# shangfuu/avse_challenge

Hardware: AMD Instinct MI355X
Metric: utterances/sec (3s@16kHz + 75 lip frames) (higher is better)
Workload: dtype fp32; 1 GPU; avse1 AV baseline train step (BASELINE configs[1]): HIP STFT front-end + AVNet (ResNet18 lip enc + TCN, dilated Conv2d audio net, LSTM fusion) fwd/bwd + Adam; global_batch=32, per_gpu_batch=32, seq_len=48000, stft_frames=376, lip_frames=75, lip_hw=96, parallelism=dp1, hip_graph=fwd+bwd+opt

## Files before the change

avse_challenge_amd/_lib.py:

```python
import ctypes
import os

import torch

_HERE = os.path.dirname(os.path.abspath(__file__))
LIB_PATH = os.environ.get("AVSE_HIP_LIB", os.path.join(_HERE, "libavse_hip.so"))

c_i64, c_i32, c_f32, c_vp = ctypes.c_int64, ctypes.c_int32, ctypes.c_float, ctypes.c_void_p

AVSE_F32, AVSE_BF16 = 0, 1


class ScanFwdArgs(ctypes.Structure):
    _fields_ = [
        ("batch", c_i64), ("dim", c_i64), ("seqlen", c_i64), ("dstate", c_i64),
        ("in_dtype", c_i32), ("delta_softplus", c_i32), ("reverse", c_i32),
        ("u", c_vp), ("u_bs", c_i64), ("u_ds", c_i64),
        ("delta", c_vp), ("delta_bs", c_i64), ("delta_ds", c_i64),
        ("A", c_vp),
        ("B", c_vp), ("B_bs", c_i64), ("B_ns", c_i64),
        ("C", c_vp), ("C_bs", c_i64), ("C_ns", c_i64),
        ("D", c_vp),
        ("z", c_vp), ("z_bs", c_i64), ("z_ds", c_i64),
        ("delta_bias", c_vp),
# ... 114 lines not shown
    "avse_prelu_gln_workspace_bytes": (c_i64, [c_i64, c_i64]),
    "avse_prelu_gln_fwd": (c_i32, [c_i64, c_i64, c_i64, c_vp, c_vp, c_vp, c_vp, c_f32, c_vp, c_vp, c_vp, c_vp]),
    "avse_prelu_gln_bwd": (c_i32, [c_i64, c_i64, c_i64] + [c_vp] * 11),
    "avse_prelu_gln_bwd_q": (c_i32, [c_i64, c_i64, c_i64] + [c_vp] * 7 + [c_i64] + [c_vp] * 6),
    "avse_dwconv_bwd_workspace_bytes": (c_i64, [c_i64, c_i64]),
    "avse_dwconv_fwd": (c_i32, [c_i64, c_i64, c_i64, c_i64, c_i64, c_vp, c_vp, c_vp, c_vp]),
    "avse_dwconv_bwd": (c_i32, [c_i64, c_i64, c_i64, c_i64, c_i64] + [c_vp] * 7),
    "avse_dwconv_gln_workspace_bytes": (c_i64, [c_i64, c_i64]),
    "avse_dwconv_gln_fwd": (c_i32, [c_i64] * 5 + [c_vp] * 5 + [c_f32] + [c_vp] * 5),
    "avse_dwconv_gln_fwd_q": (c_i32, [c_i64] * 5 + [c_vp] * 5 + [c_f32] + [c_vp] * 3 + [c_i64] + [c_vp] * 4),
    "avse_dwconv_gln_bwd": (c_i32, [c_i64] * 5 + [c_vp] * 14),
    "avse_lstm_padded_hidden": (c_i64, [c_i64]),
    "avse_lstm_group_size": (c_i64, [c_i64, c_i64]),
    "avse_lstm_group_workspace_bytes": (c_i64, [c_i64, c_i64]),
    "avse_lstm_group_capacity": (c_i64, [c_i64, c_i32]),
    "avse_lstm_fwd_group": (c_i32, [c_i64, c_i64, c_i64, c_i32, c_vp, c_vp, c_vp, c_i64, c_i64, c_vp, c_vp, c_vp, c_vp,
                                    c_vp]),
    "avse_lstm_bwd_group": (c_i32, [c_i64, c_i64, c_i64, c_i32, c_vp, c_i64, c_i64, c_vp, c_vp, c_vp, c_vp, c_vp, c_vp,
                                    c_vp]),
    "avse_lstm_fwd": (c_i32, [c_i64, c_i64, c_i64, c_i32, c_vp, c_vp, c_vp, c_i64, c_i64, c_vp, c_vp, c_vp]),
    "avse_lstm_bwd": (c_i32, [c_i64, c_i64, c_i64, c_i32, c_vp, c_i64, c_i64, c_vp, c_vp, c_vp, c_vp, c_vp]),
    "avse_gemm_bf16": (c_i32, [ctypes.POINTER(GemmBf16Args), c_vp]),
    "avse_gemm_f32s": (c_i32, [ctypes.POINTER(GemmF32sArgs), c_vp]),
    "avse_split16_planes": (c_i32, [c_i64, c_i64, c_i64, c_vp, c_i64, c_i64, c_vp, c_vp, c_vp, c_vp]),
    "avse_add_max": (c_i32, [c_i64, c_i64, c_i64, c_vp, c_vp, c_vp, c_vp, c_vp]),
    "avse_split16_planes_known": (c_i32, [c_i64, c_i64, c_i64, c_vp, c_i64, c_i64, c_vp, c_vp, c_vp, c_vp]),
    "avse_split16_planes_to": (c_i32, [c_i64, c_i64, c_i64, c_vp, c_i64, c_i64, c_vp, c_vp, c_i64, c_i64, c_vp, c_i32,
                                       c_vp]),
    "avse_dconv_wprep_bytes": (c_i64, []),
    "avse_split16": (c_i32, [c_i64, c_vp, c_vp, c_vp, c_vp]),
    "avse_split16_known": (c_i32, [c_i64, c_vp, c_vp, c_vp, c_vp]),
    "avse_dconv_wprep": (c_i32, [c_vp, c_i32, c_vp, c_vp, c_vp]),
    "avse_dconv_fwd": (c_i32, [c_i64, c_i64, c_i64, c_i64, c_vp, c_vp, c_vp, c_vp, c_vp, c_vp]),
    "avse_dconv_wgrad16_workspace_bytes": (c_i64, [c_i64, c_i64, c_i64]),
    "avse_dconv_wgrad16": (c_i32, [c_i64, c_i64, c_i64, c_i64, c_vp, c_vp, c_vp, c_vp, c_vp, c_vp, c_vp, c_vp]),
    "avse_conv1_fwd": (c_i32, [c_i64] * 3 + [c_vp] * 5),
    "avse_conv1_dgrad": (c_i32, [c_i64] * 3 + [c_vp] * 4),
    "avse_conv1_wgrad_workspace_bytes": (c_i64, [c_i64] * 3),
    "avse_conv1_wgrad": (c_i32, [c_i64] * 3 + [c_vp] * 6),
    "avse_convf_fwd": (c_i32, [c_i64] + [c_vp] * 5),
    "avse_convf_dgrad": (c_i32, [c_i64] + [c_vp] * 4),
    "avse_convf_wgrad_workspace_bytes": (c_i64, [c_i64]),
    "avse_convf_wgrad": (c_i32, [c_i64] + [c_vp] * 6),
    "avse_sconv_wprep_bytes": (c_i64, [c_i64, c_i64]),
    "avse_sconv_wprep": (c_i32, [c_i64, c_i64, c_vp, c_i32, c_vp, c_vp, c_vp]),
    "avse_sconv_fwd": (c_i32, [c_i64] * 6 + [c_vp] * 6),
    "avse_sconv_wgrad_workspace_bytes": (c_i64, [c_i64] * 6),
    "avse_sconv_wgrad": (c_i32, [c_i64] * 6 + [c_vp] * 7),
    "avse_sconv_dgrad2_supported": (c_i32, [c_i64] * 5),
    "avse_sconv_dgrad2": (c_i32, [c_i64] * 5 + [c_vp] * 6),
}

_lib = None


class HipLibraryError(RuntimeError):
    pass


ABI_VERSION = 2


def lib():
    global _lib
    if _lib is None:
        if not os.path.exists(LIB_PATH):
# ... 30 lines not shown
```

avse_challenge_amd/csrc/dconv.hip:

```cpp
#include <algorithm>

#include "common.h"

namespace avse {
namespace dcf {

typedef _Float16 half8 __attribute__((ext_vector_type(8)));
typedef float floatx16 __attribute__((ext_vector_type(16)));
typedef int i4_t __attribute__((ext_vector_type(4)));
typedef __attribute__((address_space(3))) void lds_void_t;

constexpr int C = 64, KS = 5, NQ = 4, TP = 256, THREADS = 256, WAVES = THREADS / 64;
constexpr int ROWB = 64;
constexpr int WIMG = KS * C * ROWB;
constexpr int NSTG = KS * NQ;
constexpr int MAXD = 16;
constexpr int XIMG_MAX = (TP + 8 * MAXD) * ROWB;
constexpr int STAGE = XIMG_MAX + WIMG;
constexpr int NBUF = 3;
constexpr int MAXP = (XIMG_MAX + WIMG) / 1024 / WAVES + 1;
static_assert(NBUF * STAGE <= 160 * 1024, "LDS");

__device__ inline int swz(int r) { return (r >> 2) & 3; }

// ... 457 lines not shown
        d[0] = uint4{hi[0], hi[1], hi[2], hi[3]};
        d[1] = uint4{hi[4], hi[5], hi[6], hi[7]};
        d[2] = uint4{lo[0], lo[1], lo[2], lo[3]};
        d[3] = uint4{lo[4], lo[5], lo[6], lo[7]};
    }
}

__global__ __launch_bounds__(1024) void wprep_kernel(const float* w, int transposed, uint32_t* maxbits, uint16_t* wq) {
    __shared__ uint32_t red[16];
    constexpr int TOT = C * C * KS * KS;
    float m = 0.f;
    for (int i = threadIdx.x; i < TOT; i += blockDim.x) m = fmaxf(m, fabsf(w[i]));
    uint32_t b = __float_as_uint(m);
    for (int o = 32; o >= 1; o >>= 1) b = max(b, (uint32_t)__shfl_xor((int)b, o, 64));
    if ((threadIdx.x & 63) == 0) red[threadIdx.x >> 6] = b;
    __syncthreads();
    b = 0;
    for (int k = 0; k < (int)(blockDim.x >> 6); ++k) b = max(b, red[k]);
    if (threadIdx.x == 0) maxbits[1] = b;
    const float sc = __builtin_ldexpf(1.f, split_exp(b));
    for (int e = threadIdx.x; e < TOT; e += blockDim.x) {
        const int c = e % 16, o = (e / 16) % C, kw = (e / (16 * C)) % KS, s = e / (16 * C * KS);
        const int kh = s / NQ, q = s % NQ, i = q * 16 + c;
        const float v = transposed ? w[((i * C + o) * KS + (KS - 1 - kh)) * KS + (KS - 1 - kw)]
                                   : w[((o * C + i) * KS + kh) * KS + kw];
        const float sv = v * sc;
        const _Float16 h = (_Float16)sv, l = (_Float16)(sv - (float)h);
        const int64_t row = ((int64_t)s * KS + kw) * C + o;
        wq[row * 32 + c] = __builtin_bit_cast(uint16_t, h);
        wq[row * 32 + 16 + c] = __builtin_bit_cast(uint16_t, l);
    }
}

}
}

using namespace avse::dcf;

extern "C" {

int64_t avse_dconv_wprep_bytes(void) { return (int64_t)NSTG * WIMG; }

int avse_split16(int64_t n_pix, const float* x, void* xq, uint32_t* maxbits, avse_stream_t stream) {
    if (!x || !xq || !maxbits) return AVSE_EINVAL;
    if (n_pix <= 0) return AVSE_ESHAPE;
    if (((uintptr_t)x & 15) || ((uintptr_t)xq & 15)) return AVSE_EALIGN;
    hipStream_t st = (hipStream_t)stream;
    if (hipMemsetAsync(maxbits, 0, 4, st) != hipSuccess) return AVSE_ELAUNCH;
    const int64_t n4 = n_pix * C / 4;
    hipLaunchKernelGGL(absmax_kernel, dim3((unsigned)std::max<int64_t>(1, std::min<int64_t>(AMAX_GRID, (n4 + AMAX_NT - 1) / AMAX_NT))),
                       dim3(AMAX_NT), 0, st, reinterpret_cast<const float4*>(x), n4, maxbits);
    AVSE_CHECK_LAUNCH();
    const int64_t nq = n_pix * NQ;
    const int blocks = (int)std::min<int64_t>((nq + 255) / 256, 8192);
    hipLaunchKernelGGL(split_kernel, dim3(blocks), dim3(256), 0, st, x, nq, maxbits, reinterpret_cast<uint4*>(xq));
    AVSE_CHECK_LAUNCH();
    return AVSE_OK;
}

int avse_split16_known(int64_t n_pix, const float* x, void* xq, const uint32_t* maxbits, avse_stream_t stream) {
    if (!x || !xq || !maxbits) return AVSE_EINVAL;
    if (n_pix <= 0) return AVSE_ESHAPE;
    if (((uintptr_t)x & 15) || ((uintptr_t)xq & 15)) return AVSE_EALIGN;
    const int64_t nq = n_pix * NQ;
    const int blocks = (int)std::min<int64_t>((nq + 255) / 256, 8192);
    hipLaunchKernelGGL(split_kernel, dim3(blocks), dim3(256), 0, (hipStream_t)stream, x, nq, maxbits,
                       reinterpret_cast<uint4*>(xq));
    AVSE_CHECK_LAUNCH();
    return AVSE_OK;
}

int avse_dconv_wprep(const float* w, int32_t transposed, void* wq, uint32_t* maxbits, avse_stream_t stream) {
    if (!w || !wq || !maxbits) return AVSE_EINVAL;
    hipLaunchKernelGGL(wprep_kernel, dim3(1), dim3(1024), 0, (hipStream_t)stream, w, transposed, maxbits,
                       reinterpret_cast<uint16_t*>(wq));
    AVSE_CHECK_LAUNCH();
    return AVSE_OK;
}

int64_t avse_dconv_wgrad16_workspace_bytes(int64_t N, int64_t H, int64_t W) {
    const int64_t chunks = N * ((H * W + WG_CHUNK - 1) / WG_CHUNK);
    return 4 * 2 * (int64_t)wgrad_ranges((int)std::min<int64_t>(chunks, 1 << 30)) * (KS * KS * C * C + C);
}

int avse_dconv_wgrad16(int64_t N, int64_t H, int64_t W, int64_t dil, const void* xq, const uint32_t* xmax,
                       const void* dyq, const uint32_t* dymax, float* dw, float* db, float* workspace,
                       avse_stream_t stream) {
    if (!xq || !xmax || !dyq || !dymax || !dw || !workspace) return AVSE_EINVAL;
    if (N <= 0 || H <= 0 || W < WG_CHUNK || (dil != 2 && dil != 4 && dil != 8 && dil != 16)) return AVSE_ESHAPE;
    if (N * H * W * 256 >= (1LL << 31) - 1024) return AVSE_ESHAPE;
    WArgs a;
    a.xq = xq;
    a.dyq = dyq;
    a.xmax = xmax;
    a.dymax = dymax;
    a.N = (int)N;
    a.H = (int)H;
    a.W = (int)W;
    a.cpi = (int)((H * W + WG_CHUNK - 1) / WG_CHUNK);
    a.chunks = (int)(N * a.cpi);
    a.ranges = wgrad_ranges(a.chunks);
    a.part = workspace;
    a.dbpart = db ? workspace + (int64_t)2 * a.ranges * KS * KS * C * C : nullptr;
    const dim3 grid((unsigned)(a.ranges * KS)), block(WTHREADS);
    hipStream_t st = (hipStream_t)stream;
    switch (dil) {
        case 2: hipLaunchKernelGGL(wgrad_kernel<2>, grid, block, 0, st, a); break;
        case 4: hipLaunchKernelGGL(wgrad_kernel<4>, grid, block, 0, st, a); break;
// ... 41 lines not shown
```

avse_challenge_amd/csrc/projgemm.hip:

```cpp
#include <algorithm>

#include "common.h"

namespace avse {
namespace pg {

typedef __bf16 bf16x8 __attribute__((ext_vector_type(8)));
typedef short s4_t __attribute__((ext_vector_type(4)));
typedef short s8_t __attribute__((ext_vector_type(8)));
typedef float floatx16 __attribute__((ext_vector_type(16)));
typedef __attribute__((address_space(3))) void lds_void_t;
typedef __attribute__((address_space(3))) s4_t lds_s4_t;

constexpr int BT = 256, THREADS = 512, WAVES = THREADS / 64;
constexpr int BK = 32;
constexpr int IMG = BT * BK * 2;
constexpr int STAGE = 2 * IMG;
constexpr int NBUF = 4, AHEAD = NBUF - 1;
constexpr int LWAVES = 4;
constexpr int PIECES = IMG / 1024 / LWAVES;
constexpr int LOADS = 2 * PIECES;
constexpr int RB = 2 * BK, CPR = BK / 8, RPL = 256 / RB;
static_assert(NBUF * STAGE <= 160 * 1024, "LDS");
static_assert(AHEAD >= 2 && AHEAD <= 4, "ring depth: stage s + 1 is issued before iteration s");
// ... 396 lines not shown
                            } else if (p + 7 < a.mp) {
                                reinterpret_cast<uint2*>(dst)[0] = uint2{v.x, v.y};
                                reinterpret_cast<uint2*>(dst)[1] = uint2{v.z, v.w};
                            } else {
                                const uint32_t u[4] = {v.x, v.y, v.z, v.w};
#pragma unroll
                                for (int e = 0; e < 8; ++e)
                                    if (p + e < a.mp) dst[e] = (uint16_t)(u[e >> 1] >> (16 * (e & 1)));
                            }
                        }
                    }
                    asm volatile("s_waitcnt lgkmcnt(0)" ::: "memory");
                }
            }
        }
#pragma unroll
        for (int i = 0; i < 4; ++i)
#pragma unroll
            for (int j = 0; j < 2; ++j)
#pragma unroll
                for (int e = 0; e < 16; ++e) acc[i][j][e] = 0.f;
    }
}

}
}

using namespace avse::pg;

struct PlanesArgs {
    const float* x;
    int64_t rows, r, c, bs, rs, hbs, hrs;
    int rpb;
    uint32_t* maxbits;
    _Float16* hi;
    _Float16* lo;
};

__device__ inline int64_t planes_row_off(const PlanesArgs& a, int64_t row) { return (row / a.r) * a.bs + (row % a.r) * a.rs; }
__device__ inline int64_t planes_out_off(const PlanesArgs& a, int64_t row) {
    return (row / a.r) * a.hbs + (row % a.r) * a.hrs;
}

constexpr int AM_NT = 1024, AM_GRID = 256;
template <bool VEC>
__global__ __launch_bounds__(AM_NT) void planes_absmax_kernel(PlanesArgs a, int64_t nrb) {
    __shared__ uint32_t red[AM_NT / 64];
    float m = 0.f;
    const int64_t c4 = VEC ? a.c / 4 : 0;
    for (int64_t rb = blockIdx.x; rb < nrb; rb += gridDim.x)
    for (int rr = 0; rr < a.rpb; ++rr) {
        const int64_t row = rb * a.rpb + rr;
        if (row >= a.rows) break;
        const float* xr = a.x + planes_row_off(a, row);
        if constexpr (VEC) {
            for (int64_t j0 = threadIdx.x; j0 < c4; j0 += 4 * AM_NT) {
                float4 v[4];
#pragma unroll
                for (int u = 0; u < 4; ++u)
                    v[u] = j0 + u * AM_NT < c4 ? reinterpret_cast<const float4*>(xr)[j0 + u * AM_NT] : make_float4(0.f, 0.f, 0.f, 0.f);
#pragma unroll
                for (int u = 0; u < 4; ++u)
                    m = fmaxf(m, fmaxf(fmaxf(fabsf(v[u].x), fabsf(v[u].y)), fmaxf(fabsf(v[u].z), fabsf(v[u].w))));
            }
        }
        for (int64_t i0 = 4 * c4 + threadIdx.x; i0 < a.c; i0 += 4 * AM_NT) {
            float v[4];
#pragma unroll
            for (int u = 0; u < 4; ++u) v[u] = i0 + u * AM_NT < a.c ? xr[i0 + u * AM_NT] : 0.f;
#pragma unroll
            for (int u = 0; u < 4; ++u) m = fmaxf(m, fabsf(v[u]));
        }
    }
    uint32_t v = __float_as_uint(m);
    for (int o = 32; o >= 1; o >>= 1) v = max(v, (uint32_t)__shfl_xor((int)v, o, 64));
    if ((threadIdx.x & 63) == 0) red[threadIdx.x >> 6] = v;
    __syncthreads();
    if (threadIdx.x == 0) {
        for (int k = 1; k < AM_NT / 64; ++k) v = max(v, red[k]);
        v = max(v, red[0]);
        if (v) atomicMax(a.maxbits, v);
    }
}

__device__ inline uint32_t split_pair(float x0, float x1, float sc, uint32_t& lo) {
    const float s0 = x0 * sc, s1 = x1 * sc;
    const _Float16 h0 = (_Float16)s0, h1 = (_Float16)s1;
    const _Float16 l0 = (_Float16)(s0 - (float)h0), l1 = (_Float16)(s1 - (float)h1);
    lo = (uint32_t)__builtin_bit_cast(uint16_t, l0) | ((uint32_t)__builtin_bit_cast(uint16_t, l1) << 16);
    return (uint32_t)__builtin_bit_cast(uint16_t, h0) | ((uint32_t)__builtin_bit_cast(uint16_t, h1) << 16);
}

template <bool VEC>
__global__ __launch_bounds__(256) void planes_split_kernel(PlanesArgs a) {
    const float sc = __builtin_ldexpf(1.f, split_exp_pg(*a.maxbits));
    const int64_t c4 = VEC ? a.c / 4 : 0;
    for (int rr = 0; rr < a.rpb; ++rr) {
        const int64_t row = (int64_t)blockIdx.x * a.rpb + rr;
        if (row >= a.rows) break;
        const int64_t off = planes_out_off(a, row);
        const float* xr = a.x + planes_row_off(a, row);
        if constexpr (VEC) {
            uint2* hr = reinterpret_cast<uint2*>(a.hi + off);
            uint2* lr = reinterpret_cast<uint2*>(a.lo + off);
            for (int64_t j0 = threadIdx.x; j0 < c4; j0 += 4 * 256) {
                float4 v[4];
#pragma unroll
                for (int u = 0; u < 4; ++u)
                    if (j0 + u * 256 < c4) v[u] = reinterpret_cast<const float4*>(xr)[j0 + u * 256];
#pragma unroll
                for (int u = 0; u < 4; ++u) {
                    if (j0 + u * 256 >= c4) break;
                    uint2 h, l;
                    h.x = split_pair(v[u].x, v[u].y, sc, l.x);
                    h.y = split_pair(v[u].z, v[u].w, sc, l.y);
// ... 222 lines not shown
    if (!g) return AVSE_EINVAL;
    return launch_gemm<false>(g->batch, g->mp, g->mq, g->k, g->fold, g->p, nullptr, g->p_bs, g->p_sx, g->p_sk,
                              g->p_extent, nullptr, g->q, nullptr, g->q_bs, g->q_sx, g->q_sk, g->q_extent, nullptr, g->c,
                              g->c_bs, g->c_sq, g->alpha, g->c_dtype, stream);
}

int avse_gemm_f32s(const avse_gemm_f32s_args* g, avse_stream_t stream) {
    if (!g) return AVSE_EINVAL;
    return launch_gemm<true>(g->batch, g->mp, g->mq, g->k, g->fold, g->p_hi, g->p_lo, g->p_bs, g->p_sx, g->p_sk,
                             g->p_extent, g->p_max, g->q_hi, g->q_lo, g->q_bs, g->q_sx, g->q_sk, g->q_extent, g->q_max,
                             g->c, g->c_bs, g->c_sq, g->alpha, AVSE_F32, stream, g->nsub, g->p_bs2, g->q_bs2);
}

static int split16_planes_impl(int64_t b, int64_t r, int64_t c, const float* x, int64_t x_bs, int64_t x_rs, void* hi,
                               void* lo, int64_t h_bs, int64_t h_rs, uint32_t* maxbits, bool known,
                               avse_stream_t stream, bool zero_pad = false) {
    if (!x || !hi || !lo || !maxbits) return AVSE_EINVAL;
    if (b <= 0 || r <= 0 || c <= 0 || x_rs < c || (b > 1 && x_bs < (r - 1) * x_rs + c)) return AVSE_ESHAPE;
    if (h_rs < c || (b > 1 && h_bs < (r - 1) * h_rs + c)) return AVSE_ESHAPE;
    hipStream_t st = (hipStream_t)stream;
    if (!known && hipMemsetAsync(maxbits, 0, 4, st) != hipSuccess) return AVSE_ELAUNCH;
    PlanesArgs a;
    a.x = x;
    a.rows = b * r;
    a.r = r;
    a.c = c;
    a.bs = x_bs;
    a.rs = x_rs;
    a.hbs = h_bs;
    a.hrs = h_rs;
    a.maxbits = maxbits;
    a.hi = (_Float16*)hi;
    a.lo = (_Float16*)lo;
    const int64_t c4 = (c + 3) / 4;
    a.rpb = (int)std::max<int64_t>(1, std::min<int64_t>(1024 / std::max<int64_t>(c4, 1), 64));
    const int64_t blocks = (a.rows + a.rpb - 1) / a.rpb;
    if (blocks >= (1LL << 31)) return AVSE_ESHAPE;
    const bool xvec = ((uintptr_t)x % 16 == 0) && (x_rs % 4 == 0) && (b == 1 || x_bs % 4 == 0);
    const bool hvec = ((uintptr_t)hi % 8 == 0) && ((uintptr_t)lo % 8 == 0) && (h_rs % 4 == 0) && (b == 1 || h_bs % 4 == 0);
    const bool pad = hvec && (h_rs != x_rs || (b > 1 && h_bs != x_bs) || (zero_pad && h_rs > c));
    if (!known) {
        const int64_t n = b * r * c;
        if (xvec) {
            hipLaunchKernelGGL(planes_absmax_kernel<true>, dim3((unsigned)std::min<int64_t>(blocks, AM_GRID)), dim3(AM_NT), 0,
                               st, a, blocks);
            AVSE_CHECK_LAUNCH();
        } else if (x_rs == c && (b == 1 || x_bs == r * c) && ((uintptr_t)x % 16 == 0) && n >= 4096) {
            PlanesArgs f = a;
            f.rows = f.r = n / 4096;
            f.c = f.rs = 4096;
            f.bs = 0;
            f.rpb = 1;
            hipLaunchKernelGGL(planes_absmax_kernel<true>, dim3((unsigned)std::min<int64_t>(f.rows, AM_GRID)), dim3(AM_NT), 0,
                               st, f, f.rows);
            AVSE_CHECK_LAUNCH();
            if (n % 4096) {
                f.x = x + f.rows * 4096;
                f.rows = f.r = 1;
                f.c = f.rs = n % 4096;
                hipLaunchKernelGGL(planes_absmax_kernel<false>, dim3(1), dim3(AM_NT), 0, st, f, (int64_t)1);
                AVSE_CHECK_LAUNCH();
            }
        } else {
            hipLaunchKernelGGL(planes_absmax_kernel<false>, dim3((unsigned)std::min<int64_t>(blocks, AM_GRID)), dim3(AM_NT), 0,
                               st, a, blocks);
            AVSE_CHECK_LAUNCH();
        }
    }
    if (pad) {
        PlanesArgs p2 = a;
        p2.rpb = (int)std::max<int64_t>(1, std::min<int64_t>(1024 / std::max<int64_t>(h_rs / 4, 1), 64));
        const int64_t pblocks = (a.rows + p2.rpb - 1) / p2.rpb;
        if (pblocks >= (1LL << 31)) return AVSE_ESHAPE;
        hipLaunchKernelGGL(planes_split_pad_kernel, dim3((unsigned)pblocks), dim3(256), 0, st, p2);
    } else if (xvec && hvec) {
        const int64_t n = b * r * c;
        const bool flat = x_rs == c && h_rs == c && (b == 1 || (x_bs == r * c && h_bs == r * c));
        if (flat && c < 1024 && n >= 4096) {
            PlanesArgs f = a;
            f.rows = f.r = n / 4096;
            f.c = f.rs = f.hrs = 4096;
            f.bs = f.hbs = 0;
            f.rpb = 1;
            hipLaunchKernelGGL(planes_split_kernel<true>, dim3((unsigned)f.rows), dim3(256), 0, st, f);
            if (n % 4096) {
                AVSE_CHECK_LAUNCH();
                f.x = x + f.rows * 4096;
                f.hi = a.hi + f.rows * 4096;
                f.lo = a.lo + f.rows * 4096;
                f.rows = f.r = 1;
                f.c = f.rs = f.hrs = n % 4096;
                hipLaunchKernelGGL(planes_split_kernel<true>, dim3(1), dim3(256), 0, st, f);
            }
        } else {
            hipLaunchKernelGGL(planes_split_kernel<true>, dim3((unsigned)blocks), dim3(256), 0, st, a);
        }
    } else {
        hipLaunchKernelGGL(planes_split_kernel<false>, dim3((unsigned)blocks), dim3(256), 0, st, a);
    }
    AVSE_CHECK_LAUNCH();
// ... 43 lines not shown
```

avse_challenge_amd/kernels.py:

```python
import functools

import torch

from . import _lib
from ._lib import AVSE_BF16, AVSE_F32, ScanBwdArgs, ScanFwdArgs, check, ptr, stream_ptr

NSTATE = 16

LAUNCH_TAPS = {}
LAUNCH_WORK = {}


def _tap_begin(name, device):
    taps = LAUNCH_TAPS.get(name)
    if taps is None or torch.cuda.is_current_stream_capturing():
        return None
    e0, e1 = torch.cuda.Event(enable_timing=True), torch.cuda.Event(enable_timing=True)
    e0.record(torch.cuda.current_stream(device))
    return taps, e0, e1, device, name


def _tap_end(tap, work=None):
    if tap is not None:
        taps, e0, e1, device, name = tap
# ... 451 lines not shown

def dconv_split_ok(x, dilation):
    return (x.is_cuda and x.dtype == torch.float32 and x.dim() == 4 and x.shape[1] == 64 and x.shape[3] >= 256
            and dilation in DCONV_DILATIONS and x.shape[0] * x.shape[2] * x.shape[3] * 256 < (1 << 31) - 1024)


def split16(x, maxbits):
    _need_gpu(x)
    known = _known_absmax(x)
    if is_split_q(x):
        maxbits[:1].copy_(known)
        return q_view(x)
    x = x.contiguous(memory_format=torch.channels_last)
    npix = x.shape[0] * x.shape[2] * x.shape[3]
    xq = torch.empty((npix, 256), device=x.device, dtype=torch.uint8)
    if known is not None:
        maxbits[:1].copy_(known)
        check(_lib.lib().avse_split16_known(npix, ptr(x), ptr(xq), ptr(maxbits), stream_ptr(x.device)),
              "avse_split16_known")
    else:
        check(_lib.lib().avse_split16(npix, ptr(x), ptr(xq), ptr(maxbits), stream_ptr(x.device)), "avse_split16")
    return xq


def dconv_wprep(w, transposed, maxbits):
    _need_gpu(w)
    L = _lib.lib()
    wq = torch.empty(int(L.avse_dconv_wprep_bytes()), device=w.device, dtype=torch.uint8)
    check(L.avse_dconv_wprep(ptr(w.float().contiguous()), int(bool(transposed)), ptr(wq), ptr(maxbits),
                             stream_ptr(w.device)), "avse_dconv_wprep")
    return wq


def dconv_fwd(x, w, dilation, bias=None, transposed=False, split=None):
    _need_gpu(x, w, bias)
    if not dconv_split_ok(x, dilation) or tuple(w.shape) != (64, 64, 5, 5):
        raise RuntimeError(f"dconv_fwd: unsupported shape {tuple(x.shape)} / {tuple(w.shape)} dilation {dilation}")
    N, _, H, W = x.shape
    if split is None:
        maxbits = torch.empty(2, device=x.device, dtype=torch.int32)
        xq = split16(x, maxbits)
    else:
        xq, maxbits = split
    wq = dconv_wprep(w, transposed, maxbits)
    y = torch.empty((N, 64, H, W), device=x.device, dtype=torch.float32, memory_format=torch.channels_last)
    tap = _tap_begin("avse_dconv_fwd", x.device)
    check(_lib.lib().avse_dconv_fwd(N, H, W, dilation, ptr(xq), ptr(wq), ptr(maxbits),
                                    ptr(None if bias is None else bias.float().contiguous()), ptr(y),
                                    stream_ptr(x.device)), "avse_dconv_fwd")
    _tap_end(tap)
    return y


def dconv_wgrad16(xs, dys, shape, dilation, bias_grad=False):
    (xq, xm), (dyq, dym) = xs, dys
    _need_gpu(xq, dyq)
    N, _, H, W = shape
    L = _lib.lib()
    dw = torch.empty((64, 64, 5, 5), device=xq.device, dtype=torch.float32)
    db = torch.empty(64, device=xq.device, dtype=torch.float32) if bias_grad else None
    ws = torch.empty((L.avse_dconv_wgrad16_workspace_bytes(N, H, W) + 3) // 4, device=xq.device, dtype=torch.float32)
    tap = _tap_begin("avse_dconv_wgrad16", xq.device)
    check(L.avse_dconv_wgrad16(N, H, W, dilation, ptr(xq), ptr(xm), ptr(dyq), ptr(dym), ptr(dw), ptr(db), ptr(ws),
                               stream_ptr(xq.device)), "avse_dconv_wgrad16")
    _tap_end(tap)
    return (dw, db) if bias_grad else dw



def conv1_fwd(x, w, b=None):
    _need_gpu(x, w, b)
    n, _, h, wd = x.shape
    y = torch.empty((n, 64, h, wd), device=x.device, dtype=torch.float32, memory_format=torch.channels_last)
    tap = _tap_begin("avse_conv1_fwd", x.device)
    check(_lib.lib().avse_conv1_fwd(n, h, wd, ptr(x.contiguous()), ptr(w.float().contiguous()),
                                    ptr(None if b is None else b.float().contiguous()), ptr(y), stream_ptr(x.device)),
          "avse_conv1_fwd")
# ... 928 lines not shown
```

avse_challenge_amd/layers.py:

```python

import torch
import torch.nn as nn
import torch.nn.functional as F

from . import kernels as K


class _PReLUFn(torch.autograd.Function):
    @staticmethod
    def forward(ctx, x, a):
        ctx.save_for_backward(x, a)
        return K.prelu_fwd(x, a)

    @staticmethod
    def backward(ctx, dy):
        x, a = ctx.saved_tensors
        dx, da = K.prelu_bwd(x, a, dy)
        return dx, da


class PReLU(nn.Module):
    def __init__(self, num_parameters=1, init=0.25):
        super().__init__()
        self.num_parameters = num_parameters
# ... 123 lines not shown
            else:
                dw = torch.nn.grad.conv3d_weight(x.float(), w.shape, dy, ctx.stride, ctx.padding)
        return dx, dw, None, None


class LipConv3d(nn.Conv3d):
    def __init__(self, cin, cout, kernel_size, stride=(1, 2, 2), padding=(2, 3, 3), bias=False):
        super().__init__(cin, cout, kernel_size, stride=stride, padding=padding, bias=bias)
        assert tuple(self.stride) == (1, 2, 2) and cout == 64 and not bias

    def forward(self, x):
        return _LipConv3dFn.apply(x, self.weight, tuple(self.stride), tuple(self.padding))


def _conv2d_dgrad(x, w, dy, stride, padding, dilation):
    pair = lambda v: [v, v] if isinstance(v, int) else list(v)
    return torch.ops.aten.convolution_backward(dy, x, w, None, pair(stride), pair(padding), pair(dilation), False,
                                               [0, 0], 1, [True, False, False])[0]




class _DilatedConvFn(torch.autograd.Function):

    @staticmethod
    def forward(ctx, x, w, b, dilation, add_bias):
        ctx.dilation = dilation
        ctx.split = K.dconv_split_ok(x, dilation)
        if K.is_split_q(x) and not ctx.split:
            raise RuntimeError("_DilatedConvFn: a split-output input needs the split path (DilatedConv2d.q_ok)")
        if ctx.split:
            mb = torch.empty(2, device=x.device, dtype=torch.int32)
            xq = K.split16(x, mb)
            y = K.dconv_fwd(x, w, dilation, b if add_bias else None, split=(xq, mb))
            ctx.save_for_backward(xq, mb, w)
            ctx.shape = tuple(x.shape)
            return y
        ctx.save_for_backward(x, w)
        pad = 2 * dilation
        return F.conv2d(x, w, b if add_bias else None, 1, pad, dilation)

    @staticmethod
    def backward(ctx, dy):
        d = ctx.dilation
        dx = dw = db = None
        if ctx.split:
            xq, mb, w = ctx.saved_tensors
            mbd = torch.empty(2, device=dy.device, dtype=torch.int32)
            dyq = K.split16(dy, mbd)
            if ctx.needs_input_grad[0]:
                dx = K.dconv_fwd(dy, w, d, transposed=True, split=(dyq, mbd))
            if ctx.needs_input_grad[1] or ctx.needs_input_grad[2]:
                dw, db = K.dconv_wgrad16((xq, mb[:1]), (dyq, mbd[:1]), ctx.shape, d, bias_grad=True)
                dw = dw if ctx.needs_input_grad[1] else None
                db = db if ctx.needs_input_grad[2] else None
            return dx, dw, db, None, None
        x, w = ctx.saved_tensors
        if ctx.needs_input_grad[0]:
            dx = _conv2d_dgrad(x, w, dy, 1, 2 * d, d)
        if ctx.needs_input_grad[1] and ctx.needs_input_grad[2]:
            dw, db = K.dconv_wgrad(x, dy, d, bias_grad=True)
        elif ctx.needs_input_grad[1]:
            dw = K.dconv_wgrad(x, dy, d)
        elif ctx.needs_input_grad[2]:
            db = dy.sum((0, 2, 3))
        return dx, dw, db, None, None


class _FramesNHWC(torch.autograd.Function):

    @staticmethod
    def forward(ctx, x):
        B, C, T, H, W = x.shape
        ctx.shape = x.shape
        y = K.transpose_cp(x.contiguous().view(B, C, T * H * W))
        return y.view(B * T, H, W, C).permute(0, 3, 1, 2)

    @staticmethod
    def backward(ctx, dy):
        B, C, T, H, W = ctx.shape
        d = dy.permute(0, 2, 3, 1).contiguous().view(B, T * H * W, C)
        return K.transpose_cp(d).view(B, C, T, H, W)


# ... 416 lines not shown
```

include/avse_hip.h:

```cpp
#ifndef AVSE_HIP_H
#define AVSE_HIP_H

#include <stdint.h>

#ifdef __cplusplus
extern "C" {
#endif

typedef void* avse_stream_t;

enum { AVSE_OK = 0, AVSE_EINVAL = -1, AVSE_ESHAPE = -2, AVSE_EDTYPE = -3, AVSE_ELAUNCH = -4, AVSE_EALIGN = -5,
       AVSE_ENORESIDENT = -6 };
enum { AVSE_F32 = 0, AVSE_BF16 = 1, AVSE_U8 = 2 };

const char* avse_strerror(int code);
int avse_abi_version(void);

typedef struct {
    int64_t batch, dim, seqlen, dstate;
    int32_t in_dtype;
    int32_t delta_softplus;
    int32_t reverse;
    const void* u;      int64_t u_bs, u_ds;
    const void* delta;  int64_t delta_bs, delta_ds;
// ... 206 lines not shown

typedef struct {
    int64_t batch, mp, mq, k, fold;
    const void* p;  int64_t p_bs, p_sx, p_sk, p_extent;
    const void* q;  int64_t q_bs, q_sx, q_sk, q_extent;
    void* c;        int64_t c_bs, c_sq;
    float alpha;
    int32_t c_dtype;
} avse_gemm_bf16_args;
int avse_gemm_bf16(const avse_gemm_bf16_args* a, avse_stream_t stream);

typedef struct {
    int64_t batch, mp, mq, k, fold;
    const void* p_hi; const void* p_lo;  int64_t p_bs, p_sx, p_sk, p_extent;  const uint32_t* p_max;
    const void* q_hi; const void* q_lo;  int64_t q_bs, q_sx, q_sk, q_extent;  const uint32_t* q_max;
    float* c;       int64_t c_bs, c_sq;
    float alpha;
    int64_t nsub, p_bs2, q_bs2;
} avse_gemm_f32s_args;
int avse_gemm_f32s(const avse_gemm_f32s_args* a, avse_stream_t stream);
int avse_split16_planes(int64_t b, int64_t r, int64_t c, const float* x, int64_t x_bs, int64_t x_rs, void* hi, void* lo,
                        uint32_t* maxbits, avse_stream_t stream);
int avse_add_max(int64_t rows, int64_t lp, int64_t l, const float* a, const float* b, float* y, uint32_t* maxbits,
                 avse_stream_t stream);
int avse_split16_planes_known(int64_t b, int64_t r, int64_t c, const float* x, int64_t x_bs, int64_t x_rs, void* hi,
                              void* lo, const uint32_t* maxbits, avse_stream_t stream);
int avse_split16_planes_to(int64_t b, int64_t r, int64_t c, const float* x, int64_t x_bs, int64_t x_rs, void* hi,
                           void* lo, int64_t h_bs, int64_t h_rs, uint32_t* maxbits, int32_t known, avse_stream_t stream);

int64_t avse_dconv_wprep_bytes(void);
int avse_split16(int64_t n_pix, const float* x, void* xq, uint32_t* maxbits, avse_stream_t stream);
int avse_split16_known(int64_t n_pix, const float* x, void* xq, const uint32_t* maxbits, avse_stream_t stream);
int avse_dconv_wprep(const float* w, int32_t transposed, void* wq, uint32_t* maxbits, avse_stream_t stream);

int avse_conv1_fwd(int64_t N, int64_t H, int64_t W, const float* x, const float* w, const float* b, float* y,
                   avse_stream_t stream);
int avse_conv1_dgrad(int64_t N, int64_t H, int64_t W, const float* dy, const float* w, float* dx, avse_stream_t stream);
int64_t avse_conv1_wgrad_workspace_bytes(int64_t N, int64_t H, int64_t W);
int avse_conv1_wgrad(int64_t N, int64_t H, int64_t W, const float* x, const float* dy, float* dw, float* db,
                     float* workspace, avse_stream_t stream);
int avse_convf_fwd(int64_t npix, const float* x, const float* w, const float* b, float* y, avse_stream_t stream);
int avse_convf_dgrad(int64_t npix, const float* dy, const float* w, float* dx, avse_stream_t stream);
int64_t avse_convf_wgrad_workspace_bytes(int64_t npix);
int avse_convf_wgrad(int64_t npix, const float* x, const float* dy, float* dw, float* db, float* workspace,
                     avse_stream_t stream);

int64_t avse_sconv_wprep_bytes(int64_t co, int64_t ci);
int avse_sconv_wprep(int64_t co, int64_t ci, const float* w, int32_t transposed, void* wq, uint32_t* wmax,
                     avse_stream_t stream);
int avse_sconv_fwd(int64_t N, int64_t Hi, int64_t Wi, int64_t ci, int64_t co, int64_t stride, const void* xq,
                   const uint32_t* xmax, const void* wq, const uint32_t* wmax, float* y, avse_stream_t stream);
int64_t avse_sconv_wgrad_workspace_bytes(int64_t N, int64_t Hi, int64_t Wi, int64_t ci, int64_t co, int64_t stride);
int avse_sconv_dgrad2_supported(int64_t N, int64_t Hi, int64_t Wi, int64_t ci, int64_t co);
int avse_sconv_dgrad2(int64_t N, int64_t Hi, int64_t Wi, int64_t ci, int64_t co, const void* dyq,
                      const uint32_t* dymax, const void* wq, const uint32_t* wmax, float* dx, avse_stream_t stream);
int avse_sconv_wgrad(int64_t N, int64_t Hi, int64_t Wi, int64_t ci, int64_t co, int64_t stride, const void* xq,
                     const uint32_t* xmax, const void* dyq, const uint32_t* dymax, float* dw, float* workspace,
                     avse_stream_t stream);
int avse_dconv_fwd(int64_t N, int64_t H, int64_t W, int64_t dil, const void* xq, const void* wq,
                   const uint32_t* maxbits, const float* bias, float* y, avse_stream_t stream);
int64_t avse_dconv_wgrad16_workspace_bytes(int64_t N, int64_t H, int64_t W);
int avse_dconv_wgrad16(int64_t N, int64_t H, int64_t W, int64_t dil, const void* xq, const uint32_t* xmax,
                       const void* dyq, const uint32_t* dymax, float* dw, float* db, float* workspace,
                       avse_stream_t stream);

#ifdef __cplusplus
// ... 4 lines not shown
```

Baseline: 430.8 utt/s.

## Parallelise dconv weight prep across blocks and rework planes absmax kernel

Adds a multi-block weight-prep kernel that prepares both the forward and the transposed (dgrad) split-fp16 weight images in one launch, using NSTG or 2*NSTG blocks instead of a single 1024-thread block. The transposed image is computed during forward and saved for backward, which removes a separate single-block prep launch there. Separately, the planes absmax path gains a flat vectorised kernel for contiguous inputs and a threads-per-row mapping for strided inputs, so short rows no longer leave most threads idle. Each block redundantly recomputes the full weight absmax, and the transposed weight image is kept alive from forward to backward, which costs extra memory.

Result: faster. 439.1 utt/s, median of 6 (+1.9%).

```diff
diff --git a/avse_challenge_amd/_lib.py b/avse_challenge_amd/_lib.py
--- a/avse_challenge_amd/_lib.py
+++ b/avse_challenge_amd/_lib.py
@@ -170,6 +170,7 @@
     "avse_split16_known": (c_i32, [c_i64, c_vp, c_vp, c_vp, c_vp]),
     "avse_dconv_wprep": (c_i32, [c_vp, c_i32, c_vp, c_vp, c_vp]),
     "avse_dconv_fwd": (c_i32, [c_i64, c_i64, c_i64, c_i64, c_vp, c_vp, c_vp, c_vp, c_vp, c_vp]),
+    "avse_dconv_wprep2": (c_i32, [c_vp] * 6),
     "avse_dconv_wgrad16_workspace_bytes": (c_i64, [c_i64, c_i64, c_i64]),
     "avse_dconv_wgrad16": (c_i32, [c_i64, c_i64, c_i64, c_i64, c_vp, c_vp, c_vp, c_vp, c_vp, c_vp, c_vp, c_vp]),
     "avse_conv1_fwd": (c_i32, [c_i64] * 3 + [c_vp] * 5),
diff --git a/avse_challenge_amd/csrc/dconv.hip b/avse_challenge_amd/csrc/dconv.hip
--- a/avse_challenge_amd/csrc/dconv.hip
+++ b/avse_challenge_amd/csrc/dconv.hip
@@ -513,6 +513,39 @@
     }
 }
 
+__global__ __launch_bounds__(1024) void wprep2_kernel(const float* w, uint32_t* mb0, uint32_t* mb1, uint16_t* wq0,
+                                                      uint16_t* wq1) {
+    __shared__ uint32_t red[16];
+    constexpr int TOT = C * C * KS * KS, PER = KS * C * 16;
+    float m = 0.f;
+    for (int i = threadIdx.x; i < TOT; i += 1024) m = fmaxf(m, fabsf(w[i]));
+    uint32_t b = __float_as_uint(m);
+    for (int o = 32; o >= 1; o >>= 1) b = max(b, (uint32_t)__shfl_xor((int)b, o, 64));
+    if ((threadIdx.x & 63) == 0) red[threadIdx.x >> 6] = b;
+    __syncthreads();
+    b = 0;
+    for (int k = 0; k < 16; ++k) b = max(b, red[k]);
+    if (blockIdx.x == 0 && threadIdx.x == 0) {
+        mb0[1] = b;
+        if (mb1) mb1[1] = b;
+    }
+    const float sc = __builtin_ldexpf(1.f, split_exp(b));
+    const int transposed = blockIdx.x / NSTG, s = blockIdx.x % NSTG;
+    uint16_t* wq = transposed ? wq1 : wq0;
+    const int kh = s / NQ, q = s % NQ;
+    for (int e = threadIdx.x; e < PER; e += 1024) {
+        const int c = e % 16, o = (e / 16) % C, kw = e / (16 * C);
+        const int i = q * 16 + c;
+        const float v = transposed ? w[((i * C + o) * KS + (KS - 1 - kh)) * KS + (KS - 1 - kw)]
+                                   : w[((o * C + i) * KS + kh) * KS + kw];
+        const float sv = v * sc;
+        const _Float16 h = (_Float16)sv, l = (_Float16)(sv - (float)h);
+        const int64_t row = ((int64_t)s * KS + kw) * C + o;
+        wq[row * 32 + c] = __builtin_bit_cast(uint16_t, h);
+        wq[row * 32 + 16 + c] = __builtin_bit_cast(uint16_t, l);
+    }
+}
+
 }
 }
 
@@ -555,6 +588,15 @@
     if (!w || !wq || !maxbits) return AVSE_EINVAL;
     hipLaunchKernelGGL(wprep_kernel, dim3(1), dim3(1024), 0, (hipStream_t)stream, w, transposed, maxbits,
                        reinterpret_cast<uint16_t*>(wq));
+    AVSE_CHECK_LAUNCH();
+    return AVSE_OK;
+}
+
+int avse_dconv_wprep2(const float* w, void* wq, void* wq_t, uint32_t* maxbits, uint32_t* maxbits_t,
+                      avse_stream_t stream) {
+    if (!w || !wq || !maxbits || (wq_t == nullptr) != (maxbits_t == nullptr)) return AVSE_EINVAL;
+    hipLaunchKernelGGL(wprep2_kernel, dim3(wq_t ? 2 * NSTG : NSTG), dim3(1024), 0, (hipStream_t)stream, w, maxbits,
+                       maxbits_t, reinterpret_cast<uint16_t*>(wq), reinterpret_cast<uint16_t*>(wq_t));
     AVSE_CHECK_LAUNCH();
     return AVSE_OK;
 }
diff --git a/avse_challenge_amd/csrc/projgemm.hip b/avse_challenge_amd/csrc/projgemm.hip
--- a/avse_challenge_amd/csrc/projgemm.hip
+++ b/avse_challenge_amd/csrc/projgemm.hip
@@ -452,6 +452,7 @@
     const float* x;
     int64_t rows, r, c, bs, rs, hbs, hrs;
     int rpb;
+    int tpr;
     uint32_t* maxbits;
     _Float16* hi;
     _Float16* lo;
@@ -463,35 +464,8 @@
 }
 
 constexpr int AM_NT = 1024, AM_GRID = 256;
-template <bool VEC>
-__global__ __launch_bounds__(AM_NT) void planes_absmax_kernel(PlanesArgs a, int64_t nrb) {
-    __shared__ uint32_t red[AM_NT / 64];
-    float m = 0.f;
-    const int64_t c4 = VEC ? a.c / 4 : 0;
-    for (int64_t rb = blockIdx.x; rb < nrb; rb += gridDim.x)
-    for (int rr = 0; rr < a.rpb; ++rr) {
-        const int64_t row = rb * a.rpb + rr;
-        if (row >= a.rows) break;
-        const float* xr = a.x + planes_row_off(a, row);
-        if constexpr (VEC) {
-            for (int64_t j0 = threadIdx.x; j0 < c4; j0 += 4 * AM_NT) {
-                float4 v[4];
-#pragma unroll
-                for (int u = 0; u < 4; ++u)
-                    v[u] = j0 + u * AM_NT < c4 ? reinterpret_cast<const float4*>(xr)[j0 + u * AM_NT] : make_float4(0.f, 0.f, 0.f, 0.f);
-#pragma unroll
-                for (int u = 0; u < 4; ++u)
-                    m = fmaxf(m, fmaxf(fmaxf(fabsf(v[u].x), fabsf(v[u].y)), fmaxf(fabsf(v[u].z), fabsf(v[u].w))));
-            }
-        }
-        for (int64_t i0 = 4 * c4 + threadIdx.x; i0 < a.c; i0 += 4 * AM_NT) {
-            float v[4];
-#pragma unroll
-            for (int u = 0; u < 4; ++u) v[u] = i0 + u * AM_NT < a.c ? xr[i0 + u * AM_NT] : 0.f;
-#pragma unroll
-            for (int u = 0; u < 4; ++u) m = fmaxf(m, fabsf(v[u]));
-        }
-    }
+
+__device__ inline void absmax_publish(float m, uint32_t* red, uint32_t* maxbits) {
     uint32_t v = __float_as_uint(m);
     for (int o = 32; o >= 1; o >>= 1) v = max(v, (uint32_t)__shfl_xor((int)v, o, 64));
     if ((threadIdx.x & 63) == 0) red[threadIdx.x >> 6] = v;
@@ -499,8 +473,58 @@
     if (threadIdx.x == 0) {
         for (int k = 1; k < AM_NT / 64; ++k) v = max(v, red[k]);
         v = max(v, red[0]);
-        if (v) atomicMax(a.maxbits, v);
-    }
+        if (v) atomicMax(maxbits, v);
+    }
+}
+
+template <bool VEC>
+__global__ __launch_bounds__(AM_NT) void planes_absmax_kernel(PlanesArgs a, int64_t nrb) {
+    __shared__ uint32_t red[AM_NT / 64];
+    float m = 0.f;
+    const int64_t c4 = VEC ? a.c / 4 : 0;
+    const int tpr = a.tpr, sub = threadIdx.x / tpr, tc = threadIdx.x % tpr, nsub = AM_NT / tpr;
+    for (int64_t rb = blockIdx.x; rb < nrb; rb += gridDim.x)
+    for (int rr = sub; rr < a.rpb; rr += nsub) {
+        const int64_t row = rb * a.rpb + rr;
+        if (row >= a.rows) break;
+        const float* xr = a.x + planes_row_off(a, row);
+        if constexpr (VEC) {
+            for (int64_t j0 = tc; j0 < c4; j0 += 4 * tpr) {
+                float4 v[4];
+#pragma unroll
+                for (int u = 0; u < 4; ++u)
+                    v[u] = j0 + u * tpr < c4 ? reinterpret_cast<const float4*>(xr)[j0 + u * tpr] : make_float4(0.f, 0.f, 0.f, 0.f);
+#pragma unroll
+                for (int u = 0; u < 4; ++u)
+                    m = fmaxf(m, fmaxf(fmaxf(fabsf(v[u].x), fabsf(v[u].y)), fmaxf(fabsf(v[u].z), fabsf(v[u].w))));
+            }
+        }
+        for (int64_t i0 = 4 * c4 + tc; i0 < a.c; i0 += 4 * tpr) {
+            float v[4];
+#pragma unroll
+            for (int u = 0; u < 4; ++u) v[u] = i0 + u * tpr < a.c ? xr[i0 + u * tpr] : 0.f;
+#pragma unroll
+            for (int u = 0; u < 4; ++u) m = fmaxf(m, fabsf(v[u]));
+        }
+    }
+    absmax_publish(m, red, a.maxbits);
+}
+
+__global__ __launch_bounds__(AM_NT) void planes_absmax_flat_kernel(const float* x, int64_t n, uint32_t* maxbits) {
+    __shared__ uint32_t red[AM_NT / 64];
+    float m = 0.f;
+    const int64_t n4 = n / 4, stride = (int64_t)gridDim.x * AM_NT;
+    const float4* x4 = reinterpret_cast<const float4*>(x);
+    for (int64_t i0 = blockIdx.x * (int64_t)AM_NT + threadIdx.x; i0 < n4; i0 += 4 * stride) {
+        float4 v[4];
+#pragma unroll
+        for (int u = 0; u < 4; ++u) v[u] = i0 + u * stride < n4 ? x4[i0 + u * stride] : make_float4(0.f, 0.f, 0.f, 0.f);
+#pragma unroll
+        for (int u = 0; u < 4; ++u)
+            m = fmaxf(m, fmaxf(fmaxf(fabsf(v[u].x), fabsf(v[u].y)), fmaxf(fabsf(v[u].z), fabsf(v[u].w))));
+    }
+    if (blockIdx.x == 0 && 4 * n4 + threadIdx.x < n) m = fmaxf(m, fabsf(x[4 * n4 + threadIdx.x]));
+    absmax_publish(m, red, maxbits);
 }
 
 __device__ inline uint32_t split_pair(float x0, float x1, float sc, uint32_t& lo) {
@@ -789,6 +813,7 @@
     a.maxbits = maxbits;
     a.hi = (_Float16*)hi;
     a.lo = (_Float16*)lo;
+    a.tpr = AM_NT;
     const int64_t c4 = (c + 3) / 4;
     a.rpb = (int)std::max<int64_t>(1, std::min<int64_t>(1024 / std::max<int64_t>(c4, 1), 64));
     const int64_t blocks = (a.rows + a.rpb - 1) / a.rpb;
@@ -798,31 +823,21 @@
     const bool pad = hvec && (h_rs != x_rs || (b > 1 && h_bs != x_bs) || (zero_pad && h_rs > c));
     if (!known) {
         const int64_t n = b * r * c;
-        if (xvec) {
-            hipLaunchKernelGGL(planes_absmax_kernel<true>, dim3((unsigned)std::min<int64_t>(blocks, AM_GRID)), dim3(AM_NT), 0,
-                               st, a, blocks);
-            AVSE_CHECK_LAUNCH();
-        } else if (x_rs == c && (b == 1 || x_bs == r * c) && ((uintptr_t)x % 16 == 0) && n >= 4096) {
-            PlanesArgs f = a;
-            f.rows = f.r = n / 4096;
-            f.c = f.rs = 4096;
-            f.bs = 0;
-            f.rpb = 1;
-            hipLaunchKernelGGL(planes_absmax_kernel<true>, dim3((unsigned)std::min<int64_t>(f.rows, AM_GRID)), dim3(AM_NT), 0,
-                               st, f, f.rows);
-            AVSE_CHECK_LAUNCH();
-            if (n % 4096) {
-                f.x = x + f.rows * 4096;
-                f.rows = f.r = 1;
-                f.c = f.rs = n % 4096;
-                hipLaunchKernelGGL(planes_absmax_kernel<false>, dim3(1), dim3(AM_NT), 0, st, f, (int64_t)1);
-                AVSE_CHECK_LAUNCH();
-            }
+        if (x_rs == c && (b == 1 || x_bs == r * c) && ((uintptr_t)x % 16 == 0)) {
+            const int64_t wgs = std::max<int64_t>(1, std::min<int64_t>(AM_GRID, (n / 4 + AM_NT - 1) / AM_NT));
+            hipLaunchKernelGGL(planes_absmax_flat_kernel, dim3((unsigned)wgs), dim3(AM_NT), 0, st, x, n, maxbits);
         } else {
-            hipLaunchKernelGGL(planes_absmax_kernel<false>, dim3((unsigned)std::min<int64_t>(blocks, AM_GRID)), dim3(AM_NT), 0,
-                               st, a, blocks);
-            AVSE_CHECK_LAUNCH();
-        }
+            const int64_t per_row = xvec ? c4 : c;
+            a.tpr = 1;
+            while (a.tpr < AM_NT && a.tpr < per_row) a.tpr <<= 1;
+            if (xvec)
+                hipLaunchKernelGGL(planes_absmax_kernel<true>, dim3((unsigned)std::min<int64_t>(blocks, AM_GRID)),
+                                   dim3(AM_NT), 0, st, a, blocks);
+            else
+                hipLaunchKernelGGL(planes_absmax_kernel<false>, dim3((unsigned)std::min<int64_t>(blocks, AM_GRID)),
+                                   dim3(AM_NT), 0, st, a, blocks);
+        }
+        AVSE_CHECK_LAUNCH();
     }
     if (pad) {
         PlanesArgs p2 = a;
diff --git a/avse_challenge_amd/kernels.py b/avse_challenge_amd/kernels.py
--- a/avse_challenge_amd/kernels.py
+++ b/avse_challenge_amd/kernels.py
@@ -507,7 +507,19 @@
     return wq
 
 
-def dconv_fwd(x, w, dilation, bias=None, transposed=False, split=None):
+def dconv_wprep2(w, maxbits, maxbits_t=None):
+    _need_gpu(w)
+    L = _lib.lib()
+    nb = int(L.avse_dconv_wprep_bytes())
+    wq = torch.empty(nb, device=w.device, dtype=torch.uint8)
+    wq_t = torch.empty(nb, device=w.device, dtype=torch.uint8) if maxbits_t is not None else None
+    check(L.avse_dconv_wprep2(ptr(w.float().contiguous()), ptr(wq), ptr(wq_t) if wq_t is not None else None,
+                              ptr(maxbits), ptr(maxbits_t) if maxbits_t is not None else None, stream_ptr(w.device)),
+          "avse_dconv_wprep2")
+    return wq, wq_t
+
+
+def dconv_fwd(x, w, dilation, bias=None, transposed=False, split=None, wq=None):
     _need_gpu(x, w, bias)
     if not dconv_split_ok(x, dilation) or tuple(w.shape) != (64, 64, 5, 5):
         raise RuntimeError(f"dconv_fwd: unsupported shape {tuple(x.shape)} / {tuple(w.shape)} dilation {dilation}")
@@ -517,7 +529,8 @@
         xq = split16(x, maxbits)
     else:
         xq, maxbits = split
-    wq = dconv_wprep(w, transposed, maxbits)
+    if wq is None:
+        wq = dconv_wprep(w, transposed, maxbits)
     y = torch.empty((N, 64, H, W), device=x.device, dtype=torch.float32, memory_format=torch.channels_last)
     tap = _tap_begin("avse_dconv_fwd", x.device)
     check(_lib.lib().avse_dconv_fwd(N, H, W, dilation, ptr(xq), ptr(wq), ptr(maxbits),
diff --git a/avse_challenge_amd/layers.py b/avse_challenge_amd/layers.py
--- a/avse_challenge_amd/layers.py
+++ b/avse_challenge_amd/layers.py
@@ -179,8 +179,14 @@
         if ctx.split:
             mb = torch.empty(2, device=x.device, dtype=torch.int32)
             xq = K.split16(x, mb)
-            y = K.dconv_fwd(x, w, dilation, b if add_bias else None, split=(xq, mb))
-            ctx.save_for_backward(xq, mb, w)
+            mbd = torch.empty(2, device=x.device, dtype=torch.int32) if ctx.needs_input_grad[0] else None
+            wq, wq_t = K.dconv_wprep2(w, mb, mbd)
+            y = K.dconv_fwd(x, w, dilation, b if add_bias else None, split=(xq, mb), wq=wq)
+            ctx.has_wt = wq_t is not None
+            if ctx.has_wt:
+                ctx.save_for_backward(xq, mb, w, wq_t, mbd)
+            else:
+                ctx.save_for_backward(xq, mb, w)
             ctx.shape = tuple(x.shape)
             return y
         ctx.save_for_backward(x, w)
@@ -192,11 +198,14 @@
         d = ctx.dilation
         dx = dw = db = None
         if ctx.split:
-            xq, mb, w = ctx.saved_tensors
-            mbd = torch.empty(2, device=dy.device, dtype=torch.int32)
+            if ctx.has_wt:
+                xq, mb, w, wq_t, mbd = ctx.saved_tensors
+            else:
+                xq, mb, w = ctx.saved_tensors
+                wq_t, mbd = None, torch.empty(2, device=dy.device, dtype=torch.int32)
             dyq = K.split16(dy, mbd)
             if ctx.needs_input_grad[0]:
-                dx = K.dconv_fwd(dy, w, d, transposed=True, split=(dyq, mbd))
+                dx = K.dconv_fwd(dy, w, d, transposed=True, split=(dyq, mbd), wq=wq_t)
             if ctx.needs_input_grad[1] or ctx.needs_input_grad[2]:
                 dw, db = K.dconv_wgrad16((xq, mb[:1]), (dyq, mbd[:1]), ctx.shape, d, bias_grad=True)
                 dw = dw if ctx.needs_input_grad[1] else None
diff --git a/include/avse_hip.h b/include/avse_hip.h
--- a/include/avse_hip.h
+++ b/include/avse_hip.h
@@ -262,6 +262,8 @@
 int avse_split16(int64_t n_pix, const float* x, void* xq, uint32_t* maxbits, avse_stream_t stream);
 int avse_split16_known(int64_t n_pix, const float* x, void* xq, const uint32_t* maxbits, avse_stream_t stream);
 int avse_dconv_wprep(const float* w, int32_t transposed, void* wq, uint32_t* maxbits, avse_stream_t stream);
+int avse_dconv_wprep2(const float* w, void* wq, void* wq_t, uint32_t* maxbits, uint32_t* maxbits_t,
+                      avse_stream_t stream);
 
 int avse_conv1_fwd(int64_t N, int64_t H, int64_t W, const float* x, const float* w, const float* b, float* y,
                    avse_stream_t stream);
```
